# awslabs/dgl-ke

Hardware: NVIDIA H100
Metric: edges/sec TransE_l2 d=400 neg=200 at 1/2/4/8 H100 vs ref CPU; HBM GB/s %peak (higher is better)
Workload: dtype f32

## Files before the change

dgl-ke_b200/csrc/kge_fused.cu:

```cuda
#include <cuda.h>
#include <cstdio>
#include <cstdlib>
#include "kge_common.cuh"
#include "kge_tc.cuh"

namespace kge {

using namespace tc;

namespace {

constexpr int kTileM = 128;
constexpr int kThreadsF = 384;
constexpr int kProducerWarp = 8;
constexpr int kMaxS1 = 4, kMaxS2 = 8;
constexpr int kMaxPf = 8;
constexpr uint32_t kRingBytes = 192 * 1024;
constexpr int kWc = 128;
constexpr float kLog2e = 1.4426950408889634f;
constexpr float kLn2 = 0.6931471805599453f;

struct FusedArgs {
  int model, adversarial;
  float gamma, Tl2e, inv2B, uni;
  float reg_coef;
  int reg_norm;
  int C, Rx, Ry, D;
  int N1;
  int nblkD;
  int nS1, nS2;
  uint32_t stage1Bytes, stage2Bytes;
  float *VhiT, *VloT;
  float* colpart;
  int ncolpart;
  const float* x2;
  const float* y2;
  const float* pos;
  const float* wt;
  const float* wbar;
  float *gpos, *rowsum, *pl, *nl;
  float* dumpS;
  float* dumpV;
  const float *Xhi, *Xlo;
  const long long* xids;
  TableView xtab;
  const float* xraw;
  float* gsn;
  float* out;
  int pf_slots;
  int pf_parity;
  int pf_lag;
// ... 43 lines not shown
  };
  for (long long k = 0; k < n && k < S; ++k) load(k);
  const int L = g.pf_lag < S - 1 ? g.pf_lag : (S > 2 ? S - 2 : 1);
  for (long long k = 0; k < n; ++k) {
    const int s = (int)(k % S);
    mbar_wait(&pf_full[w][s], (uint32_t)((k / S) & 1));
    const long long v = vrow(k);
    float* dst = v < nU ? g.pf_nc + v * (long long)g.D : g.pf_bn + (v - nU) * (long long)g.D;
    const long long kr = k - L + S;
    const bool reload = k >= L && kr < n;
    if (reload && kr >= base + 32) { base += 32; ids_lo = ids_hi; ids_hi = fetch_ids(base + 32); }
    if (elect_one()) {
      bulk_s2g(dst, slots + (size_t)s * g.pf_row_bytes, g.pf_row_bytes);
      bulk_commit();
      if (reload) { if (L == 3) bulk_wait_read<3>(); else if (L == 2) bulk_wait_read<2>(); else bulk_wait_read<1>(); }
    }
    __syncwarp();
    if (reload) load(kr);
  }
  if (elect_one()) bulk_wait_all();
  __syncwarp();
}

template <int NV>
__global__ void __launch_bounds__(kThreadsF, 1)
k_fused_pos(const __grid_constant__ CUtensorMap mXh, const __grid_constant__ CUtensorMap mXl,
            const __grid_constant__ CUtensorMap mYh1, const __grid_constant__ CUtensorMap mYl1,
            const __grid_constant__ CUtensorMap mYh2, const __grid_constant__ CUtensorMap mYl2, FusedArgs g) {
  extern __shared__ __align__(1024) uint8_t smem_raw[];
  __shared__ __align__(8) uint64_t full1[kMaxS1], empty1[kMaxS1], full2[kMaxS2], empty2[kMaxS2];
  __shared__ __align__(8) uint64_t pf_full[2][kMaxPf];
  __shared__ __align__(16) float colA[NV];
  __shared__ __align__(16) float cpart[8][NV];

  const int warp = threadIdx.x >> 5, lane = threadIdx.x & 31;
  uint8_t* ring = (uint8_t*)(((uintptr_t)smem_raw + 1023) & ~(uintptr_t)1023);

  const int mtiles = (g.Rx + kTileM - 1) / kTileM;
  const int ntiles = g.C * mtiles;
  const int nkb1 = (g.D + 31) >> 5;
  const int nkb2 = (g.Ry + 31) >> 5;
  const int nchunks = (g.D + kWc - 1) / kWc;
  constexpr uint32_t yBytes1 = (uint32_t)NV * 128u;
  constexpr uint32_t yBytes2 = (uint32_t)kWc * 128u;
  const bool l2 = g.model == KGE_TRANSE_L2;

  if (threadIdx.x == 0) {
    for (int s = 0; s < kMaxS1; ++s) { mbar_init(&full1[s], 1); mbar_init(&empty1[s], 8); }
    for (int s = 0; s < kMaxS2; ++s) { mbar_init(&full2[s], 1); mbar_init(&empty2[s], 8); }
    for (int s = 0; s < kMaxPf; ++s) { mbar_init(&pf_full[0][s], 1); mbar_init(&pf_full[1][s], 1); }
    asm volatile("fence.mbarrier_init.release.cluster;" ::: "memory");
  }
  if (warp == kProducerWarp && lane == 0) {
    tma_prefetch_desc(&mXh); tma_prefetch_desc(&mXl); tma_prefetch_desc(&mYh1);
    tma_prefetch_desc(&mYl1); tma_prefetch_desc(&mYh2); tma_prefetch_desc(&mYl2);
  }
  __syncthreads();

  if (warp >= 8) {
  asm volatile("setmaxnreg.dec.sync.aligned.u32 56;");
  if (warp == kProducerWarp) {
    uint32_t n1 = 0, n2 = 0;
    for (int tile = blockIdx.x; tile < ntiles; tile += gridDim.x) {
      const int c = tile / mtiles, m0 = (tile % mtiles) * kTileM;
      for (uint32_t k = (n2 > (uint32_t)g.nS2 ? n2 - g.nS2 : 0); k < n2; ++k) mbar_wait(&empty2[k % g.nS2], (k / g.nS2) & 1);
      for (int kb = 0; kb < nkb1; ++kb, ++n1) {
        const uint32_t s = n1 % g.nS1;
        mbar_wait(&empty1[s], ((n1 / g.nS1) & 1) ^ 1);
        uint8_t* st = ring + (size_t)s * g.stage1Bytes;
        const int yx = (c * g.nblkD + kb) * g.Rx + m0;
        const int yy = (c * g.nblkD + kb) * g.Ry;
        if (elect_one()) {
          mbar_expect_tx(&full1[s], 2u * 16384u + 2u * yBytes1);
          tma_load_2d(st, &mXh, &full1[s], 0, yx);
          tma_load_2d(st + 16384, &mXl, &full1[s], 0, yx);
          tma_load_2d(st + 32768, &mYh1, &full1[s], 0, yy);
          tma_load_2d(st + 32768 + yBytes1, &mYl1, &full1[s], 0, yy);
        }
        __syncwarp();
      }
      for (uint32_t k = (n1 > (uint32_t)g.nS1 ? n1 - g.nS1 : 0); k < n1; ++k) mbar_wait(&empty1[k % g.nS1], (k / g.nS1) & 1);
      for (int ch = 0; ch < nchunks; ++ch) {
        for (int kb = 0; kb < nkb2; ++kb, ++n2) {
          const uint32_t s = n2 % g.nS2;
          mbar_wait(&empty2[s], ((n2 / g.nS2) & 1) ^ 1);
          uint8_t* st = ring + (size_t)s * g.stage2Bytes;
          const int yy = (c * nkb2 + kb) * g.D + ch * kWc;
          if (elect_one()) {
            mbar_expect_tx(&full2[s], 2u * yBytes2);
            tma_load_2d(st, &mYh2, &full2[s], 0, yy);
            tma_load_2d(st + yBytes2, &mYl2, &full2[s], 0, yy);
          }
          __syncwarp();
        }
      }
    }
  } else if (warp >= 10 && g.pf_slots > 0) {
    prefetch_rows(g, ring, pf_full, warp - 10, lane);
  }
  } else {
    asm volatile("setmaxnreg.inc.sync.aligned.u32 224;");
    const int wg = warp >> 2, q = lane & 3;
    const int et = threadIdx.x;
    const int rloc = wg * 64 + (warp & 3) * 16 + (lane >> 2);
    uint32_t n1 = 0, n2 = 0;
    float acc[NV / 2];
    for (int tile = blockIdx.x; tile < ntiles; tile += gridDim.x) {
      const int c = tile / mtiles, m0 = (tile % mtiles) * kTileM;
      epi_bar();
      for (int y = et; y < NV; y += 256) {
        const bool ok = y < g.Ry;
        colA[y] = (l2 && ok) ? g.y2[(long long)c * g.Ry + y] : 0.f;
      }
      epi_bar();
#pragma unroll
      for (int i = 0; i < NV / 2; ++i) acc[i] = 0.f;
      for (int kb = 0; kb < nkb1; ++kb, ++n1) {
        const uint32_t s = n1 % g.nS1;
        mbar_wait(&full1[s], (n1 / g.nS1) & 1);
        const uint32_t st = smem_u32(ring + (size_t)s * g.stage1Bytes);
        const uint64_t dXh = make_desc(st + wg * 8192u), dXl = make_desc(st + 16384u + wg * 8192u);
        const uint64_t dYh = make_desc(st + 32768u), dYl = make_desc(st + 32768u + yBytes1);
        const int kleft = g.D - kb * 32;
        const int ksteps = kleft >= 32 ? 4 : (kleft >> 3);
        wgmma_fence();
        for (int ks = 0; ks < ksteps; ++ks) {
          const uint64_t o = (uint64_t)(ks * 2);
          wgmma_ss<NV>(acc, dXh + o, dYh + o, 1u);
          wgmma_ss<NV>(acc, dXh + o, dYl + o, 1u);
          wgmma_ss<NV>(acc, dXl + o, dYh + o, 1u);
        }
        wgmma_commit();
        if (kb > 0) {
          wgmma_wait<1>();
          if (lane == 0) mbar_arrive(&empty1[(n1 - 1) % g.nS1]);
        }
      }
      wgmma_wait<0>();
      if (lane == 0) mbar_arrive(&empty1[(n1 - 1) % g.nS1]);
      reg_fence(acc);

      float rscal[2];
#pragma unroll
      for (int h = 0; h < 2; ++h) {
        const int m = m0 + rloc + 8 * h;
        const bool row_ok = m < g.Rx;
        const long long gx = (long long)c * g.Rx + (row_ok ? m : 0);
        const float x2v = (l2 && row_ok) ? g.x2[gx] : 0.f;
        const float w_i = (g.wt && row_ok) ? g.wt[gx] : 1.f;
        const float kw = w_i * g.inv2B;
        float mxl = -INFINITY;
        if (g.adversarial || g.dumpS) {
#pragma unroll
          for (int j = 0; j < NV / 8; ++j) {
            float sv[2];
#pragma unroll
            for (int e = 0; e < 2; ++e) {
              const int col = 8 * j + 2 * q + e;
              float s = acc[4 * j + 2 * h + e];
              if (l2) {
                const float sqc = fmaxf(fmaf(-2.f, s, colA[col]) + x2v, 1e-30f);
                s = g.gamma - sqc * rsqrta(sqc);
              }
              sv[e] = s;
              if (col < g.Ry) mxl = fmaxf(mxl, s * g.Tl2e);
// ... 12 lines not shown
#pragma unroll
        for (int j = 0; j < NV / 8; ++j) {
#pragma unroll
          for (int e = 0; e < 2; ++e) {
            const int col = 8 * j + 2 * q + e;
            float s = acc[4 * j + 2 * h + e], rinv = 1.f;
            if (l2) {
              const float sq = fmaf(-2.f, s, colA[col]) + x2v;
              const float sqc = fmaxf(sq, 1e-30f);
              const float r = rsqrta(sqc);
              s = g.gamma - sqc * r;
              rinv = (sq > 1e-30f) ? r : 0.f;
            }
            const float pe = g.adversarial ? ex2a(fmaf(s, g.Tl2e, -mxl)) : 1.f;
            const float t = ex2a(-fabsf(s) * kLog2e);
            const float u = 1.f + t;
            const float r1 = rcpa(u);
            const float sig = (s >= 0.f) ? r1 : t * r1;
            const float sp = fmaf(kLn2, lg2a(u), fmaxf(s, 0.f));
            const bool ok = row_ok && (col < g.Ry);
            const float coef = ok ? pe * sig * kw * rinv : 0.f;
            if (ok) { nls = fmaf(pe, sp, nls); den += pe; }
            rs += coef;
            acc[4 * j + 2 * h + e] = coef;
          }
        }
        den += __shfl_xor_sync(0xffffffffu, den, 1); den += __shfl_xor_sync(0xffffffffu, den, 2);
        nls += __shfl_xor_sync(0xffffffffu, nls, 1); nls += __shfl_xor_sync(0xffffffffu, nls, 2);
        rs += __shfl_xor_sync(0xffffffffu, rs, 1); rs += __shfl_xor_sync(0xffffffffu, rs, 2);
        const float rscale = g.adversarial ? (row_ok ? 1.f / den : 0.f) : g.uni;
        rscal[h] = rscale;
        if (g.dumpV && row_ok) {
#pragma unroll
          for (int j = 0; j < NV / 8; ++j)
            if (8 * j + 2 * q < g.Ry)
              *reinterpret_cast<float2*>(g.dumpV + gx * g.Ry + 8 * j + 2 * q) =
                  make_float2(acc[4 * j + 2 * h] * rscale, acc[4 * j + 2 * h + 1] * rscale);
        }
        {
          float* vh = g.VhiT + slabT_off(c, g.Rx, g.Ry, m, 0);
          float* vl = g.VloT + slabT_off(c, g.Rx, g.Ry, m, 0);
#pragma unroll
          for (int j = 0; j < NV / 8; ++j) {
#pragma unroll
            for (int e = 0; e < 2; ++e) {
              const int col = 8 * j + 2 * q + e;
              const float v = acc[4 * j + 2 * h + e] * rscale;
              if (row_ok && col < g.Ry) {
                float hi, lo;
                split_tf32(v, hi, lo);
                vh[col * 32] = hi; vl[col * 32] = lo;
              }
              if (l2) {
                float s = v;
                s += __shfl_xor_sync(0xffffffffu, s, 4);
                s += __shfl_xor_sync(0xffffffffu, s, 8);
                s += __shfl_xor_sync(0xffffffffu, s, 16);
                if (lane < 4) cpart[warp][col] = h ? cpart[warp][col] + s : s;
              }
            }
          }
        }
        if (q == 0 && row_ok) {
          const float ps = g.pos[gx];
          const float wb = g.wt ? *g.wbar : 1.f;
          g.pl[gx] = softplusf(-ps);
          g.nl[gx] = nls * rscale * w_i;
          g.gpos[gx] = -sigmoidf(-ps) * wb * g.inv2B;
          if (l2) g.rowsum[gx] = rs * rscale;
        }
      }
      if (l2) {
        epi_bar();
        float* dst = g.colpart + (long long)(tile % mtiles) * g.C * g.Ry + (long long)c * g.Ry;
        for (int y = et; y < g.Ry; y += 256) {
          float s = cpart[0][y];
#pragma unroll
          for (int w = 1; w < 8; ++w) s += cpart[w][y];
          dst[y] = s;
        }
      }
      {
        const int srcLo = (lane & ~3) | (q >> 1), srcHi = srcLo + 2;
        const bool odd = q & 1;
#pragma unroll
        for (int j = 0; j < NV / 8; ++j) {
          float o[4];
#pragma unroll
          for (int h = 0; h < 2; ++h) {
            const float v0 = acc[4 * j + 2 * h], v1 = acc[4 * j + 2 * h + 1];
            const float a0 = __shfl_sync(0xffffffffu, v0, srcLo), a1 = __shfl_sync(0xffffffffu, v1, srcLo);
            const float b0 = __shfl_sync(0xffffffffu, v0, srcHi), b1 = __shfl_sync(0xffffffffu, v1, srcHi);
            o[h] = odd ? a1 : a0;
            o[2 + h] = odd ? b1 : b0;
          }
          acc[4 * j + 0] = o[0]; acc[4 * j + 1] = o[1]; acc[4 * j + 2] = o[2]; acc[4 * j + 3] = o[3];
        }
      }

      for (int ch = 0; ch < nchunks; ++ch) {
        const int d0 = ch * kWc;
        float acc2[kWc / 2];
#pragma unroll
        for (int i = 0; i < kWc / 2; ++i) acc2[i] = 0.f;
#pragma unroll
        for (int kb = 0; kb < (NV + 31) / 32; ++kb) {
          if (kb >= nkb2) break;
          const uint32_t s = n2 % g.nS2;
          mbar_wait(&full2[s], (n2 / g.nS2) & 1);
          const uint32_t st = smem_u32(ring + (size_t)s * g.stage2Bytes);
          const uint64_t dYh = make_desc(st), dYl = make_desc(st + yBytes2);
          const int kleft = g.Ry - kb * 32;
          const int ksteps = kleft >= 32 ? 4 : (kleft >> 3);
          uint32_t ah[2][4] = {}, al[2][4] = {};
#pragma unroll
          for (int ks = 0; ks < 4; ++ks) {
            const int j = kb * 4 + ks;
            if (j < NV / 8 && ks < ksteps) {
              if (ks >= 2) wgmma_wait<1>();
#pragma unroll
              for (int r = 0; r < 4; ++r) {
                float hi, lo;
                split_tf32(acc[4 * j + r], hi, lo);
                ah[ks & 1][r] = __float_as_uint(hi); al[ks & 1][r] = __float_as_uint(lo);
              }
              wgmma_fence();
              const uint64_t o = (uint64_t)(ks * 2);
              wgmma_rs<kWc>(acc2, ah[ks & 1], dYh + o, 1u);
              wgmma_rs<kWc>(acc2, ah[ks & 1], dYl + o, 1u);
              wgmma_rs<kWc>(acc2, al[ks & 1], dYh + o, 1u);
              wgmma_commit();
              if (ks >= 1) { reg_fence(ah[(ks - 1) & 1]); reg_fence(al[(ks - 1) & 1]); }
            }
          }
          wgmma_wait<0>();
          reg_fence(ah[0]); reg_fence(ah[1]); reg_fence(al[0]); reg_fence(al[1]);
          if (lane == 0) mbar_arrive(&empty2[s]);
          ++n2;
        }
        reg_fence(acc2);
#pragma unroll
        for (int h = 0; h < 2; ++h) {
          const int m = m0 + rloc + 8 * h;
          if (m >= g.Rx) continue;
          float* orow = g.out + ((long long)c * g.Rx + m) * (long long)g.D;
#pragma unroll
          for (int j = 0; j < kWc / 8; ++j) {
            const int k = d0 + 8 * j + 2 * q;
            if (k >= g.D) continue;
            *reinterpret_cast<float2*>(orow + k) = make_float2(acc2[4 * j + 2 * h] * rscal[h], acc2[4 * j + 2 * h + 1] * rscal[h]);
          }
        }
      }
    }
  }
}

template <int NW, int KS>
__device__ __forceinline__ void neg_kblock(float (&acc)[NW / 2], uint64_t dVh, uint64_t dVl, uint64_t dAh, uint64_t dAl) {
  wgmma_fence();
#pragma unroll
  for (int ks = 0; ks < KS; ++ks) {
    const uint64_t o = (uint64_t)(ks * 2);
    wgmma_ss<NW>(acc, dVh + o, dAh + o, 1u);
    wgmma_ss<NW>(acc, dVh + o, dAl + o, 1u);
    wgmma_ss<NW>(acc, dVl + o, dAh + o, 1u);
  }
  wgmma_commit();
}

constexpr int kNegEpiLoads = 16;

template <int NW, bool FLAT>
__global__ void __launch_bounds__(kThreadsF, 1)
k_fused_neg(const __grid_constant__ CUtensorMap mVh, const __grid_constant__ CUtensorMap mVl,
            const __grid_constant__ CUtensorMap mAh, const __grid_constant__ CUtensorMap mAl, FusedArgs g) {
  extern __shared__ __align__(1024) uint8_t smem_raw[];
  __shared__ __align__(8) uint64_t full[kMaxS1], empty[kMaxS1];
  __shared__ __align__(8) uint64_t pf_full[2][kMaxPf];

  const int warp = threadIdx.x >> 5, lane = threadIdx.x & 31;
  uint8_t* ring = (uint8_t*)(((uintptr_t)smem_raw + 1023) & ~(uintptr_t)1023);

  const int mtiles = (g.Rx + kTileM - 1) / kTileM;
  const int ntiles = g.C * mtiles;
  const int nkb = (g.Ry + 31) >> 5;
  const int nch = (g.D + NW - 1) / NW;
  constexpr uint32_t aBytes = (uint32_t)kTileM * 128u;
  constexpr uint32_t bBytes = (uint32_t)NW * 128u;
  const bool l2 = g.model == KGE_TRANSE_L2;

// ... 86 lines not shown
            bh[jj] = __ldg(reinterpret_cast<const float2*>(brow[h] + k));
          } else {
            const long long so = boff[h] + (k >> 5) * blk + (k & 31);
            bh[jj] = __ldg(reinterpret_cast<const float2*>(g.Xhi + so));
            bl[jj] = __ldg(reinterpret_cast<const float2*>(g.Xlo + so));
          }
        }
      };
      float gsq[2] = {0.f, 0.f};
      for (int ch = 0; ch < nch; ++ch) {
        const int d0 = ch * NW;
        float acc[NW / 2];
#pragma unroll
        for (int i = 0; i < NW / 2; ++i) acc[i] = 0.f;
        for (int kb = 0; kb < nkb; ++kb, ++n) {
          const uint32_t s = n % g.nS1;
          mbar_wait(&full[s], (n / g.nS1) & 1);
          const uint32_t st = smem_u32(ring + (size_t)s * g.stage1Bytes);
          const uint64_t dVh = make_desc(st + wg * 8192u), dVl = make_desc(st + aBytes + wg * 8192u);
          const uint64_t dAh = make_desc(st + 2 * aBytes), dAl = make_desc(st + 2 * aBytes + bBytes);
          const int kleft = g.Ry - kb * 32;
          const int ksteps = kleft >= 32 ? 4 : (kleft >> 3);
          switch (ksteps) {
            case 4: neg_kblock<NW, 4>(acc, dVh, dVl, dAh, dAl); break;
            case 3: neg_kblock<NW, 3>(acc, dVh, dVl, dAh, dAl); break;
            case 2: neg_kblock<NW, 2>(acc, dVh, dVl, dAh, dAl); break;
            default: neg_kblock<NW, 1>(acc, dVh, dVl, dAh, dAl); break;
          }
          if (kb > 0) {
            wgmma_wait<1>();
            if (lane == 0) mbar_arrive(&empty[(n - 1) % g.nS1]);
          }
        }
        if (early) load_b(0, d0, 0);
        wgmma_wait<0>();
        if (lane == 0) mbar_arrive(&empty[(n - 1) % g.nS1]);
        reg_fence(acc);
#pragma unroll
        for (int h = 0; h < 2; ++h) {
          if (!rok[h]) continue;
          float* orow = g.out + ((long long)c * g.Rx + m0 + rloc + 8 * h) * (long long)g.D;
#pragma unroll
          for (int j0 = 0; j0 < NJ; j0 += NB) {
            if (!early || h > 0 || j0 > 0) load_b(h, d0, j0);
#pragma unroll
            for (int jj = 0; jj < NB; ++jj) {
              const int j = j0 + jj;
              const int k = d0 + 8 * j + 2 * q;
              if (j >= NJ || k >= g.D) continue;
              float o0 = acc[4 * j + 2 * h], o1 = acc[4 * j + 2 * h + 1];
// ... 6 lines not shown
            }
          }
        }
      }
#pragma unroll
      for (int h = 0; h < 2; ++h) {
        float v = gsq[h];
        v += __shfl_xor_sync(0xffffffffu, v, 1);
        v += __shfl_xor_sync(0xffffffffu, v, 2);
        const int m = m0 + rloc + 8 * h;
        if (q == 0 && m < g.Rx) g.gsn[(long long)c * g.Rx + m] = v / (float)g.D;
      }
    }
  }
}

}

bool fused_supported(const StepParams& p) {
  return umma_supported(p) && !p.hinge && !p.pairwise && !p.neg_deg && p.Cs <= 240 && p.Ns <= 240;
}

namespace {
struct Geometry { int Rx, Ry, N1, nS1, nS2, pf_slots; uint32_t stage1Bytes, stage2Bytes, pf_off; bool ok; };

int neg_chunk_width(int D, bool want_prefetch) {
  static const int widths[] = {64, 128, 200, 256};
  int best = 0;
  long long best_rows = 0;
  for (int w : widths) {
    if (w == 256 && want_prefetch) continue;
    const long long rows = (long long)((D + w - 1) / w) * (kTileM + w);
    if (!best || rows < best_rows) { best = w; best_rows = rows; }
  }
  return best;
}

Geometry geometry(const StepParams& p, int mode, bool want_prefetch) {
  Geometry q{};
  const uint32_t row = (uint32_t)p.D * 4u;
  if (mode == 1) {
    q.Rx = p.Ns; q.Ry = p.Cs;
    q.N1 = neg_chunk_width(p.D, want_prefetch);
    q.stage1Bytes = 2u * kTileM * 128u + 2u * (uint32_t)q.N1 * 128u;
    q.nS1 = (int)(kRingBytes / q.stage1Bytes); if (q.nS1 > kMaxS1) q.nS1 = kMaxS1;
    q.ok = q.nS1 >= 2;
    if (q.ok && want_prefetch) {
      int nS = q.nS1;
      while (nS > 2 && kRingBytes - (uint32_t)nS * q.stage1Bytes < 2u * kMaxPf * row) --nS;
      const uint32_t used = (uint32_t)nS * q.stage1Bytes;
      int slots = (int)((kRingBytes - used) / (2u * row));
      if (slots > kMaxPf) slots = kMaxPf;
      if (slots >= 2) { q.pf_slots = slots; q.nS1 = nS; q.pf_off = used; }
    }
    return q;
  }
  q.Rx = p.Cs; q.Ry = p.Ns;
  q.N1 = q.Ry <= 64 ? 64 : (q.Ry <= 128 ? 128 : (q.Ry <= 208 ? 208 : 256));
  q.stage1Bytes = 2u * 16384u + 2u * (uint32_t)q.N1 * 128u;
  q.stage2Bytes = 2u * (uint32_t)kWc * 128u;
  q.nS1 = (int)(kRingBytes / q.stage1Bytes); if (q.nS1 > kMaxS1) q.nS1 = kMaxS1;
  q.nS2 = (int)(kRingBytes / q.stage2Bytes); if (q.nS2 > kMaxS2) q.nS2 = kMaxS2;
  q.ok = q.nS1 >= 2 && q.nS2 >= 2;
  if (q.ok && want_prefetch) {
    int nS1 = q.nS1, nS2 = q.nS2;
    uint32_t want = 2u * kMaxPf * row;
    while (nS1 > 2 && kRingBytes - (uint32_t)nS1 * q.stage1Bytes < want) --nS1;
    uint32_t used = (uint32_t)nS1 * q.stage1Bytes;
    if (want > kRingBytes - used) want = kRingBytes - used;
    while (nS2 > 4 && kRingBytes - (uint32_t)nS2 * q.stage2Bytes < want) --nS2;
    if ((uint32_t)nS2 * q.stage2Bytes > used) used = (uint32_t)nS2 * q.stage2Bytes;
    int slots = (int)((kRingBytes - used) / (2u * row));
    if (slots > kMaxPf) slots = kMaxPf;
    if (slots >= 2) { q.pf_slots = slots; q.nS1 = nS1; q.nS2 = nS2; q.pf_off = used; }
  }
  return q;
}

int launch_error() {
  const cudaError_t e = cudaGetLastError();
  return e == cudaSuccess ? KGE_OK : fail(KGE_ERR_CUDA, "k_fused launch: %s", cudaGetErrorString(e));
}
template <int NV>
int launch_pos(const LaunchCtx& c, int grid, size_t smem, const CUtensorMap* m, const FusedArgs& g) {
  if (int rc = smem_optin((const void*)k_fused_pos<NV>, smem)) return rc;
  KGE_LAUNCH_NAMED(c, "k_fused<P: S=A.Bn^T, loss, GA=V.Bn>", (k_fused_pos<NV>), grid, kThreadsF, smem,
                   m[0], m[1], m[2], m[3], m[4], m[5], g);
  return launch_error();
}
template <int NW, bool FLAT>
int launch_neg_src(const LaunchCtx& c, int grid, size_t smem, const CUtensorMap* m, const FusedArgs& g) {
  if (int rc = smem_optin((const void*)k_fused_neg<NW, FLAT>, smem)) return rc;
  KGE_LAUNCH_NAMED(c, "k_fused<N: G_neg=V^T.A, mean sq>", (k_fused_neg<NW, FLAT>), grid, kThreadsF, smem, m[0], m[1], m[2], m[3], g);
  return launch_error();
}
template <int NW>
int launch_neg(const LaunchCtx& c, int grid, size_t smem, const CUtensorMap* m, const FusedArgs& g) {
  return (g.xraw || g.xids) ? launch_neg_src<NW, true>(c, grid, smem, m, g) : launch_neg_src<NW, false>(c, grid, smem, m, g);
}
int launch_width(const LaunchCtx& c, bool P, int grid, size_t smem, const CUtensorMap* m, const FusedArgs& g) {
  switch (g.N1) {
    case 64: return P ? launch_pos<64>(c, grid, smem, m, g) : launch_neg<64>(c, grid, smem, m, g);
    case 128: return P ? launch_pos<128>(c, grid, smem, m, g) : launch_neg<128>(c, grid, smem, m, g);
    case 200: return launch_neg<200>(c, grid, smem, m, g);
    case 208: return launch_pos<208>(c, grid, smem, m, g);
    default: return P ? launch_pos<256>(c, grid, smem, m, g) : launch_neg<256>(c, grid, smem, m, g);
  }
}
}

int fused_prefetch_slots(const StepParams& p, int mode) { return geometry(p, mode, true).pf_slots; }

int fused_launch(const LaunchCtx& c, const StepParams& p, const StepWs& w, int mode, const float* wt, float* dumpS,
                 float* dumpV, const TableView* ent, const long long* neg_ids, const FusedPrefetch* pf) {
  FusedArgs g{};
  g.model = p.model; g.adversarial = p.adversarial;
  g.gamma = p.gamma; g.Tl2e = p.adv_temperature * kLog2e; g.inv2B = 0.5f / (float)p.B; g.uni = 1.f / (float)p.Ns;
  g.reg_coef = p.reg_coef; g.reg_norm = p.reg_norm;
  g.C = p.C; g.D = p.D; g.nblkD = slab_blocks(p.D);
  const bool P = mode == 0;
  const Geometry q = geometry(p, mode, pf != nullptr && ent != nullptr);
  if (!q.ok) return fail(KGE_ERR_UNSUPPORTED, "fused kernel: shape does not fit (N1=%d)", q.N1);
  g.Rx = q.Rx; g.Ry = q.Ry; g.N1 = q.N1; g.nS1 = q.nS1; g.nS2 = q.nS2;
  g.stage1Bytes = q.stage1Bytes; g.stage2Bytes = q.stage2Bytes;
  if (pf && ent && q.pf_slots >= 2) {
    static const int lag_env = getenv("KGE_B200_PF_LAG") ? atoi(getenv("KGE_B200_PF_LAG")) : 1;
    g.pf_lag = lag_env < 1 ? 1 : (lag_env > 3 ? 3 : lag_env);
    g.pf_slots = q.pf_slots; g.pf_off = q.pf_off; g.pf_row_bytes = (uint32_t)p.D * 4u; g.pf_parity = mode;
    g.pf_node_ids = pf->node_ids; g.pf_nU_dev = pf->nU_dev; g.pf_nU = pf->nU; g.pf_nNeg = pf->nNeg;
    g.pf_neg_ids = pf->neg_ids; g.pf_nc = pf->nc; g.pf_bn = pf->bn;
    g.xtab = *ent;
  }
  g.VhiT = w.VhiT; g.VloT = w.VloT; g.colpart = w.colpart; g.ncolpart = (p.Cs + kTileM - 1) / kTileM;
  g.dumpV = dumpV;
  const size_t smem = kRingBytes + 1024;
  const int mtiles = (g.Rx + kTileM - 1) / kTileM;
  int grid = p.C * mtiles;
  if (grid > c.num_sms) grid = c.num_sms;
  CUtensorMap m[6];
  if (P) {
    g.x2 = w.a2; g.y2 = w.b2;
    g.pos = w.pos; g.wt = wt; g.wbar = w.wbar;
    g.gpos = w.gpos; g.rowsum = w.rowsum; g.pl = w.pl; g.nl = w.nl;
    g.dumpS = dumpS;
    g.out = w.GA;
    const long long rowsX = (long long)p.C * p.Cs * g.nblkD, rowsY = (long long)p.C * p.Ns * g.nblkD;
    const long long rowsYT = (long long)p.C * slab_blocks(p.Ns) * p.D;
    if (tc_make_map(&m[0], w.Ahi, rowsX, 32, kTileM) || tc_make_map(&m[1], w.Alo, rowsX, 32, kTileM) ||
        tc_make_map(&m[2], w.Bhi, rowsY, 32, g.N1) || tc_make_map(&m[3], w.Blo, rowsY, 32, g.N1) ||
        tc_make_map(&m[4], w.BhiT, rowsYT, 32, kWc) || tc_make_map(&m[5], w.BloT, rowsYT, 32, kWc))
      return KGE_ERR_CUDA;
    return launch_width(c, true, grid, smem, m, g);
  }
  g.Xhi = w.Bhi; g.Xlo = w.Blo;
  if (ent && ent->n_shards == 1 && neg_ids) { g.xids = neg_ids; g.xtab = *ent; }
  if (w.BnRaw) g.xraw = w.BnRaw;
  g.gsn = w.gsn;
  g.out = w.Bn;
  const long long rowsV = (long long)p.C * slab_blocks(p.Cs) * p.Ns, rowsA = (long long)p.C * slab_blocks(p.Cs) * p.D;
  if (tc_make_map(&m[0], w.VhiT, rowsV, 32, kTileM) || tc_make_map(&m[1], w.VloT, rowsV, 32, kTileM) ||
      tc_make_map(&m[2], w.AhiT, rowsA, 32, g.N1) || tc_make_map(&m[3], w.AloT, rowsA, 32, g.N1))
    return KGE_ERR_CUDA;
  return launch_width(c, false, grid, smem, m, g);
}

}
```

dgl-ke_b200/csrc/kge_tc.cuh:

```cuda
#pragma once
#include <cuda.h>
#include <cuda_runtime.h>
#include <stdint.h>

namespace kge {
namespace tc {

__device__ __forceinline__ uint32_t smem_u32(const void* p) { return (uint32_t)__cvta_generic_to_shared(p); }

__device__ __forceinline__ bool elect_one() {
  uint32_t pred = 0;
  asm volatile(
      "{\n\t.reg .pred P1;\n\t"
      "elect.sync _|P1, 0xFFFFFFFF;\n\t"
      "selp.b32 %0, 1, 0, P1;\n\t}"
      : "=r"(pred));
  return pred != 0;
}

__device__ __forceinline__ void mbar_init(uint64_t* bar, uint32_t count) {
  asm volatile("mbarrier.init.shared::cta.b64 [%0], %1;" ::"r"(smem_u32(bar)), "r"(count));
}
__device__ __forceinline__ void mbar_expect_tx(uint64_t* bar, uint32_t bytes) {
  asm volatile("mbarrier.arrive.expect_tx.shared::cta.b64 _, [%0], %1;" ::"r"(smem_u32(bar)), "r"(bytes) : "memory");
// ... 72 lines not shown
               : "l"(adesc), "l"(bdesc), "r"(accumulate));
}
template <>
__device__ __forceinline__ void wgmma_ss<208>(float (&d)[104], uint64_t adesc, uint64_t bdesc, uint32_t accumulate) {
  asm volatile("{\n\t.reg .pred p;\n\tsetp.ne.b32 p, %106, 0;\n\t"
               "wgmma.mma_async.sync.aligned.m64n208k8.f32.tf32.tf32 {%0,%1,%2,%3,%4,%5,%6,%7,%8,%9,%10,%11,%12,%13,%14,%15,%16,%17,%18,%19,%20,%21,%22,%23,%24,%25,%26,%27,%28,%29,%30,%31,%32,%33,%34,%35,%36,%37,%38,%39,%40,%41,%42,%43,%44,%45,%46,%47,%48,%49,%50,%51,%52,%53,%54,%55,%56,%57,%58,%59,%60,%61,%62,%63,%64,%65,%66,%67,%68,%69,%70,%71,%72,%73,%74,%75,%76,%77,%78,%79,%80,%81,%82,%83,%84,%85,%86,%87,%88,%89,%90,%91,%92,%93,%94,%95,%96,%97,%98,%99,%100,%101,%102,%103}, %104, %105, p, 1, 1;\n\t}"
               : KGE_D32(0), KGE_D32(32), KGE_D32(64), KGE_D4(96), KGE_D4(100)
               : "l"(adesc), "l"(bdesc), "r"(accumulate));
}
template <>
__device__ __forceinline__ void wgmma_ss<256>(float (&d)[128], uint64_t adesc, uint64_t bdesc, uint32_t accumulate) {
  asm volatile("{\n\t.reg .pred p;\n\tsetp.ne.b32 p, %130, 0;\n\t"
               "wgmma.mma_async.sync.aligned.m64n256k8.f32.tf32.tf32 {%0,%1,%2,%3,%4,%5,%6,%7,%8,%9,%10,%11,%12,%13,%14,%15,%16,%17,%18,%19,%20,%21,%22,%23,%24,%25,%26,%27,%28,%29,%30,%31,%32,%33,%34,%35,%36,%37,%38,%39,%40,%41,%42,%43,%44,%45,%46,%47,%48,%49,%50,%51,%52,%53,%54,%55,%56,%57,%58,%59,%60,%61,%62,%63,%64,%65,%66,%67,%68,%69,%70,%71,%72,%73,%74,%75,%76,%77,%78,%79,%80,%81,%82,%83,%84,%85,%86,%87,%88,%89,%90,%91,%92,%93,%94,%95,%96,%97,%98,%99,%100,%101,%102,%103,%104,%105,%106,%107,%108,%109,%110,%111,%112,%113,%114,%115,%116,%117,%118,%119,%120,%121,%122,%123,%124,%125,%126,%127}, %128, %129, p, 1, 1;\n\t}"
               : KGE_D32(0), KGE_D32(32), KGE_D32(64), KGE_D32(96)
               : "l"(adesc), "l"(bdesc), "r"(accumulate));
}
template <>
__device__ __forceinline__ void wgmma_rs<128>(float (&d)[64], const uint32_t (&a)[4], uint64_t bdesc, uint32_t accumulate) {
  asm volatile("{\n\t.reg .pred p;\n\tsetp.ne.b32 p, %69, 0;\n\t"
               "wgmma.mma_async.sync.aligned.m64n128k8.f32.tf32.tf32 {%0,%1,%2,%3,%4,%5,%6,%7,%8,%9,%10,%11,%12,%13,%14,%15,%16,%17,%18,%19,%20,%21,%22,%23,%24,%25,%26,%27,%28,%29,%30,%31,%32,%33,%34,%35,%36,%37,%38,%39,%40,%41,%42,%43,%44,%45,%46,%47,%48,%49,%50,%51,%52,%53,%54,%55,%56,%57,%58,%59,%60,%61,%62,%63}, {%64,%65,%66,%67}, %68, p, 1, 1;\n\t}"
               : KGE_D32(0), KGE_D32(32)
               : "r"(a[0]), "r"(a[1]), "r"(a[2]), "r"(a[3]), "l"(bdesc), "r"(accumulate));
}
#undef KGE_D4
#undef KGE_D16
#undef KGE_D32

__device__ __forceinline__ uint64_t make_desc(uint32_t saddr) {
  uint64_t d = 0;
  d |= (uint64_t)((saddr >> 4) & 0x3FFF);
  d |= (uint64_t)1 << 16;
  d |= (uint64_t)(1024 >> 4) << 32;
  d |= (uint64_t)1 << 62;
  return d;
}

__device__ __forceinline__ float ex2a(float x) { float y; asm("ex2.approx.ftz.f32 %0, %1;" : "=f"(y) : "f"(x)); return y; }
__device__ __forceinline__ float lg2a(float x) { float y; asm("lg2.approx.ftz.f32 %0, %1;" : "=f"(y) : "f"(x)); return y; }
__device__ __forceinline__ float rcpa(float x) { float y; asm("rcp.approx.ftz.f32 %0, %1;" : "=f"(y) : "f"(x)); return y; }
__device__ __forceinline__ float rsqrta(float x) { float y; asm("rsqrt.approx.ftz.f32 %0, %1;" : "=f"(y) : "f"(x)); return y; }
__device__ __forceinline__ float sqrta(float x) { float y; asm("sqrt.approx.ftz.f32 %0, %1;" : "=f"(y) : "f"(x)); return y; }

}

int tc_make_map(CUtensorMap* m, const float* base, long long rows, long long cols, int box_rows);

// ... 2 lines not shown
```

Measured before the change: 29.44 million.

## Stage V tile in shared memory, offload V export to handoff warps, add n200 second GEMM

The positive-side fused kernel now writes the softmax coefficient matrix V into a swizzled shared-memory buffer instead of holding it in registers. Dedicated handoff warps then export the hi/lo split of V to global memory and reduce the column sums, overlapping that work with the second GEMM. The second GEMM reads its A fragments from shared memory and can use an N=200 chunk width when that wastes less padding for D (e.g. D=400). The ring buffer grows when prefetch is off, and a vfree barrier gates reuse of the V buffer. The change adds shared-memory traffic and a new cross-warp synchronisation, and it leaves fewer pipeline stages for the V buffer.

```diff
diff --git a/dgl-ke_b200/csrc/kge_fused.cu b/dgl-ke_b200/csrc/kge_fused.cu
--- a/dgl-ke_b200/csrc/kge_fused.cu
+++ b/dgl-ke_b200/csrc/kge_fused.cu
@@ -1,6 +1,7 @@
 #include <cuda.h>
 #include <cstdio>
 #include <cstdlib>
+#include <mutex>
 #include "kge_common.cuh"
 #include "kge_tc.cuh"
 
@@ -13,10 +14,11 @@
 constexpr int kTileM = 128;
 constexpr int kThreadsF = 384;
 constexpr int kProducerWarp = 8;
+constexpr int kHandoffWarp = 9;
 constexpr int kMaxS1 = 4, kMaxS2 = 8;
 constexpr int kMaxPf = 8;
 constexpr uint32_t kRingBytes = 192 * 1024;
-constexpr int kWc = 128;
+constexpr uint32_t kRingBytesP = 223 * 1024;
 constexpr float kLog2e = 1.4426950408889634f;
 constexpr float kLn2 = 0.6931471805599453f;
 
@@ -27,6 +29,7 @@
   int reg_norm;
   int C, Rx, Ry, D;
   int N1;
+  int N2;
   int nblkD;
   int nS1, nS2;
   uint32_t stage1Bytes, stage2Bytes;
@@ -116,32 +119,83 @@
   __syncwarp();
 }
 
+template <int NW, int KS>
+__device__ __forceinline__ void kblock_3xtf32(float (&acc)[NW / 2], uint64_t dXh, uint64_t dXl, uint64_t dYh, uint64_t dYl) {
+  wgmma_fence();
+#pragma unroll
+  for (int ks = 0; ks < KS; ++ks) {
+    const uint64_t o = (uint64_t)(ks * 2);
+    wgmma_ss<NW>(acc, dXh + o, dYh + o, 1u);
+    wgmma_ss<NW>(acc, dXh + o, dYl + o, 1u);
+    wgmma_ss<NW>(acc, dXl + o, dYh + o, 1u);
+  }
+  wgmma_commit();
+}
+
 template <int NV>
+__device__ __forceinline__ int vsm_idx(int i, int k) {
+  const int g = i & 7, h = (i >> 3) & 1, kk = k & 7;
+  const int L = 4 * g + (kk & 3);
+  return (((i >> 4) * (NV / 8) + (k >> 3)) * 32 + (L ^ ((L >> 3) & 3))) * 4 + h + 2 * (kk >> 2);
+}
+
+template <int NW>
+__device__ __forceinline__ void pos_kstep(float (&acc2)[NW / 2], uint32_t (&ah)[4], uint32_t (&al)[4], const float* vf,
+                                          uint64_t dYh, uint64_t dYl) {
+  const float4 v = *reinterpret_cast<const float4*>(vf);
+  const float a[4] = {v.x, v.y, v.z, v.w};
+#pragma unroll
+  for (int r = 0; r < 4; ++r) {
+    float hi, lo;
+    split_tf32(a[r], hi, lo);
+    ah[r] = __float_as_uint(hi); al[r] = __float_as_uint(lo);
+  }
+  wgmma_fence();
+  wgmma_rs<NW>(acc2, ah, dYh, 1u);
+  wgmma_rs<NW>(acc2, ah, dYl, 1u);
+  wgmma_rs<NW>(acc2, al, dYh, 1u);
+  wgmma_commit();
+}
+
+__device__ __forceinline__ int tile_row() {
+  uint32_t t;
+  asm volatile("mov.u32 %0, %%tid.x;" : "=r"(t));
+  return (int)((t >> 5) * 16 + ((t >> 2) & 7));
+}
+
+template <int NV, int NW>
 __global__ void __launch_bounds__(kThreadsF, 1)
 k_fused_pos(const __grid_constant__ CUtensorMap mXh, const __grid_constant__ CUtensorMap mXl,
             const __grid_constant__ CUtensorMap mYh1, const __grid_constant__ CUtensorMap mYl1,
             const __grid_constant__ CUtensorMap mYh2, const __grid_constant__ CUtensorMap mYl2, FusedArgs g) {
   extern __shared__ __align__(1024) uint8_t smem_raw[];
   __shared__ __align__(8) uint64_t full1[kMaxS1], empty1[kMaxS1], full2[kMaxS2], empty2[kMaxS2];
+  __shared__ __align__(8) uint64_t vfree;
   __shared__ __align__(8) uint64_t pf_full[2][kMaxPf];
   __shared__ __align__(16) float colA[NV];
-  __shared__ __align__(16) float cpart[8][NV];
+  __shared__ float rsc[kTileM];
 
   const int warp = threadIdx.x >> 5, lane = threadIdx.x & 31;
   uint8_t* ring = (uint8_t*)(((uintptr_t)smem_raw + 1023) & ~(uintptr_t)1023);
+  float* vsm = reinterpret_cast<float*>(ring);
+  constexpr uint32_t vBytes = (uint32_t)NV * 512u;
+  uint8_t* ring2 = ring + vBytes;
 
   const int mtiles = (g.Rx + kTileM - 1) / kTileM;
   const int ntiles = g.C * mtiles;
   const int nkb1 = (g.D + 31) >> 5;
   const int nkb2 = (g.Ry + 31) >> 5;
-  const int nchunks = (g.D + kWc - 1) / kWc;
+  const int nchunks = (g.D + NW - 1) / NW;
   constexpr uint32_t yBytes1 = (uint32_t)NV * 128u;
-  constexpr uint32_t yBytes2 = (uint32_t)kWc * 128u;
+  constexpr uint32_t yBytes2 = (uint32_t)NW * 128u;
   const bool l2 = g.model == KGE_TRANSE_L2;
+  const int nhand = g.pf_slots > 0 ? 1 : 3;
+  const uint32_t hand_bar_n = 256u + 32u * (uint32_t)nhand;
 
   if (threadIdx.x == 0) {
     for (int s = 0; s < kMaxS1; ++s) { mbar_init(&full1[s], 1); mbar_init(&empty1[s], 8); }
     for (int s = 0; s < kMaxS2; ++s) { mbar_init(&full2[s], 1); mbar_init(&empty2[s], 8); }
+    mbar_init(&vfree, 8 + nhand);
     for (int s = 0; s < kMaxPf; ++s) { mbar_init(&pf_full[0][s], 1); mbar_init(&pf_full[1][s], 1); }
     asm volatile("fence.mbarrier_init.release.cluster;" ::: "memory");
   }
@@ -154,10 +208,10 @@
   if (warp >= 8) {
   asm volatile("setmaxnreg.dec.sync.aligned.u32 56;");
   if (warp == kProducerWarp) {
-    uint32_t n1 = 0, n2 = 0;
-    for (int tile = blockIdx.x; tile < ntiles; tile += gridDim.x) {
+    uint32_t n1 = 0, n2 = 0, it = 0;
+    for (int tile = blockIdx.x; tile < ntiles; tile += gridDim.x, ++it) {
       const int c = tile / mtiles, m0 = (tile % mtiles) * kTileM;
-      for (uint32_t k = (n2 > (uint32_t)g.nS2 ? n2 - g.nS2 : 0); k < n2; ++k) mbar_wait(&empty2[k % g.nS2], (k / g.nS2) & 1);
+      if (it > 0) mbar_wait(&vfree, (it - 1) & 1);
       for (int kb = 0; kb < nkb1; ++kb, ++n1) {
         const uint32_t s = n1 % g.nS1;
         mbar_wait(&empty1[s], ((n1 / g.nS1) & 1) ^ 1);
@@ -178,8 +232,8 @@
         for (int kb = 0; kb < nkb2; ++kb, ++n2) {
           const uint32_t s = n2 % g.nS2;
           mbar_wait(&empty2[s], ((n2 / g.nS2) & 1) ^ 1);
-          uint8_t* st = ring + (size_t)s * g.stage2Bytes;
-          const int yy = (c * nkb2 + kb) * g.D + ch * kWc;
+          uint8_t* st = ring2 + (size_t)s * g.stage2Bytes;
+          const int yy = (c * nkb2 + kb) * g.D + ch * NW;
           if (elect_one()) {
             mbar_expect_tx(&full2[s], 2u * yBytes2);
             tma_load_2d(st, &mYh2, &full2[s], 0, yy);
@@ -189,6 +243,43 @@
         }
       }
     }
+  } else if (warp - kHandoffWarp < nhand) {
+    const int hw = warp - kHandoffWarp;
+    for (int tile = blockIdx.x; tile < ntiles; tile += gridDim.x) {
+      const int c = tile / mtiles, m0 = (tile % mtiles) * kTileM;
+      const int rows = g.Rx - m0 < kTileM ? g.Rx - m0 : kTileM;
+      const int nb = (rows + 31) >> 5;
+      asm volatile("bar.sync 2, %0;" ::"r"(hand_bar_n) : "memory");
+      float* dst = g.colpart + (long long)(tile % mtiles) * g.C * g.Ry + (long long)c * g.Ry;
+      for (int j = hw; j < g.Ry; j += nhand) {
+        float s = 0.f;
+        float v[kTileM / 32];
+#pragma unroll
+        for (int b = 0; b < kTileM / 32; ++b) {
+          const int i = 32 * b + lane;
+          v[b] = b < nb ? vsm[vsm_idx<NV>(i, j)] * rsc[i] : 0.f;
+        }
+#pragma unroll
+        for (int b = 0; b < kTileM / 32; ++b) {
+          const int i = 32 * b + lane;
+          if (i < rows) {
+            float hi, lo;
+            split_tf32(v[b], hi, lo);
+            const long long o = slabT_off(c, g.Rx, g.Ry, m0 + i, j);
+            g.VhiT[o] = hi; g.VloT[o] = lo;
+          }
+          s += v[b];
+        }
+        if (l2) {
+#pragma unroll
+          for (int x = 16; x >= 1; x >>= 1) s += __shfl_xor_sync(0xffffffffu, s, x);
+          if (lane == 0) dst[j] = s;
+        }
+      }
+      asm volatile("fence.proxy.async.shared::cta;" ::: "memory");
+      __syncwarp();
+      if (lane == 0) mbar_arrive(&vfree);
+    }
   } else if (warp >= 10 && g.pf_slots > 0) {
     prefetch_rows(g, ring, pf_full, warp - 10, lane);
   }
@@ -196,9 +287,7 @@
     asm volatile("setmaxnreg.inc.sync.aligned.u32 224;");
     const int wg = warp >> 2, q = lane & 3;
     const int et = threadIdx.x;
-    const int rloc = wg * 64 + (warp & 3) * 16 + (lane >> 2);
     uint32_t n1 = 0, n2 = 0;
-    float acc[NV / 2];
     for (int tile = blockIdx.x; tile < ntiles; tile += gridDim.x) {
       const int c = tile / mtiles, m0 = (tile % mtiles) * kTileM;
       epi_bar();
@@ -207,6 +296,9 @@
         colA[y] = (l2 && ok) ? g.y2[(long long)c * g.Ry + y] : 0.f;
       }
       epi_bar();
+      float rscal[2];
+      {
+      float acc[NV / 2];
 #pragma unroll
       for (int i = 0; i < NV / 2; ++i) acc[i] = 0.f;
       for (int kb = 0; kb < nkb1; ++kb, ++n1) {
@@ -217,14 +309,12 @@
         const uint64_t dYh = make_desc(st + 32768u), dYl = make_desc(st + 32768u + yBytes1);
         const int kleft = g.D - kb * 32;
         const int ksteps = kleft >= 32 ? 4 : (kleft >> 3);
-        wgmma_fence();
-        for (int ks = 0; ks < ksteps; ++ks) {
-          const uint64_t o = (uint64_t)(ks * 2);
-          wgmma_ss<NV>(acc, dXh + o, dYh + o, 1u);
-          wgmma_ss<NV>(acc, dXh + o, dYl + o, 1u);
-          wgmma_ss<NV>(acc, dXl + o, dYh + o, 1u);
-        }
-        wgmma_commit();
+        switch (ksteps) {
+          case 4: kblock_3xtf32<NV, 4>(acc, dXh, dXl, dYh, dYl); break;
+          case 3: kblock_3xtf32<NV, 3>(acc, dXh, dXl, dYh, dYl); break;
+          case 2: kblock_3xtf32<NV, 2>(acc, dXh, dXl, dYh, dYl); break;
+          default: kblock_3xtf32<NV, 1>(acc, dXh, dXl, dYh, dYl); break;
+        }
         if (kb > 0) {
           wgmma_wait<1>();
           if (lane == 0) mbar_arrive(&empty1[(n1 - 1) % g.nS1]);
@@ -233,8 +323,9 @@
       wgmma_wait<0>();
       if (lane == 0) mbar_arrive(&empty1[(n1 - 1) % g.nS1]);
       reg_fence(acc);
-
-      float rscal[2];
+      epi_bar();
+      const int rloc = tile_row();
+
 #pragma unroll
       for (int h = 0; h < 2; ++h) {
         const int m = m0 + rloc + 8 * h;
@@ -293,7 +384,7 @@
             const float coef = ok ? pe * sig * kw * rinv : 0.f;
             if (ok) { nls = fmaf(pe, sp, nls); den += pe; }
             rs += coef;
-            acc[4 * j + 2 * h + e] = coef;
+            vsm[vsm_idx<NV>(rloc + 8 * h, col)] = coef;
           }
         }
         den += __shfl_xor_sync(0xffffffffu, den, 1); den += __shfl_xor_sync(0xffffffffu, den, 2);
@@ -302,35 +393,11 @@
         const float rscale = g.adversarial ? (row_ok ? 1.f / den : 0.f) : g.uni;
         rscal[h] = rscale;
         if (g.dumpV && row_ok) {
-#pragma unroll
           for (int j = 0; j < NV / 8; ++j)
             if (8 * j + 2 * q < g.Ry)
               *reinterpret_cast<float2*>(g.dumpV + gx * g.Ry + 8 * j + 2 * q) =
-                  make_float2(acc[4 * j + 2 * h] * rscale, acc[4 * j + 2 * h + 1] * rscale);
-        }
-        {
-          float* vh = g.VhiT + slabT_off(c, g.Rx, g.Ry, m, 0);
-          float* vl = g.VloT + slabT_off(c, g.Rx, g.Ry, m, 0);
-#pragma unroll
-          for (int j = 0; j < NV / 8; ++j) {
-#pragma unroll
-            for (int e = 0; e < 2; ++e) {
-              const int col = 8 * j + 2 * q + e;
-              const float v = acc[4 * j + 2 * h + e] * rscale;
-              if (row_ok && col < g.Ry) {
-                float hi, lo;
-                split_tf32(v, hi, lo);
-                vh[col * 32] = hi; vl[col * 32] = lo;
-              }
-              if (l2) {
-                float s = v;
-                s += __shfl_xor_sync(0xffffffffu, s, 4);
-                s += __shfl_xor_sync(0xffffffffu, s, 8);
-                s += __shfl_xor_sync(0xffffffffu, s, 16);
-                if (lane < 4) cpart[warp][col] = h ? cpart[warp][col] + s : s;
-              }
-            }
-          }
+                  make_float2(vsm[vsm_idx<NV>(rloc + 8 * h, 8 * j + 2 * q)] * rscale,
+                              vsm[vsm_idx<NV>(rloc + 8 * h, 8 * j + 2 * q + 1)] * rscale);
         }
         if (q == 0 && row_ok) {
           const float ps = g.pos[gx];
@@ -341,74 +408,45 @@
           if (l2) g.rowsum[gx] = rs * rscale;
         }
       }
-      if (l2) {
-        epi_bar();
-        float* dst = g.colpart + (long long)(tile % mtiles) * g.C * g.Ry + (long long)c * g.Ry;
-        for (int y = et; y < g.Ry; y += 256) {
-          float s = cpart[0][y];
-#pragma unroll
-          for (int w = 1; w < 8; ++w) s += cpart[w][y];
-          dst[y] = s;
-        }
-      }
-      {
-        const int srcLo = (lane & ~3) | (q >> 1), srcHi = srcLo + 2;
-        const bool odd = q & 1;
-#pragma unroll
-        for (int j = 0; j < NV / 8; ++j) {
-          float o[4];
-#pragma unroll
-          for (int h = 0; h < 2; ++h) {
-            const float v0 = acc[4 * j + 2 * h], v1 = acc[4 * j + 2 * h + 1];
-            const float a0 = __shfl_sync(0xffffffffu, v0, srcLo), a1 = __shfl_sync(0xffffffffu, v1, srcLo);
-            const float b0 = __shfl_sync(0xffffffffu, v0, srcHi), b1 = __shfl_sync(0xffffffffu, v1, srcHi);
-            o[h] = odd ? a1 : a0;
-            o[2 + h] = odd ? b1 : b0;
-          }
-          acc[4 * j + 0] = o[0]; acc[4 * j + 1] = o[1]; acc[4 * j + 2] = o[2]; acc[4 * j + 3] = o[3];
-        }
-      }
-
+      if (q == 0) { rsc[rloc] = rscal[0]; rsc[rloc + 8] = rscal[1]; }
+      }
+      asm volatile("bar.arrive 2, %0;" ::"r"(hand_bar_n) : "memory");
+      __syncwarp();
+
+      const float* vw = vsm + ((warp * (NV / 8)) * 32 + (lane ^ ((lane >> 3) & 3))) * 4;
+      const int rloc = tile_row();
       for (int ch = 0; ch < nchunks; ++ch) {
-        const int d0 = ch * kWc;
-        float acc2[kWc / 2];
-#pragma unroll
-        for (int i = 0; i < kWc / 2; ++i) acc2[i] = 0.f;
-#pragma unroll
-        for (int kb = 0; kb < (NV + 31) / 32; ++kb) {
-          if (kb >= nkb2) break;
+        const int d0 = ch * NW;
+        float acc2[NW / 2];
+#pragma unroll
+        for (int i = 0; i < NW / 2; ++i) acc2[i] = 0.f;
+        uint32_t ah[2][4], al[2][4];
+#pragma unroll 1
+        for (int kb = 0; kb < nkb2; ++kb) {
           const uint32_t s = n2 % g.nS2;
           mbar_wait(&full2[s], (n2 / g.nS2) & 1);
-          const uint32_t st = smem_u32(ring + (size_t)s * g.stage2Bytes);
+          const uint32_t st = smem_u32(ring2 + (size_t)s * g.stage2Bytes);
           const uint64_t dYh = make_desc(st), dYl = make_desc(st + yBytes2);
           const int kleft = g.Ry - kb * 32;
           const int ksteps = kleft >= 32 ? 4 : (kleft >> 3);
-          uint32_t ah[2][4] = {}, al[2][4] = {};
 #pragma unroll
           for (int ks = 0; ks < 4; ++ks) {
             const int j = kb * 4 + ks;
-            if (j < NV / 8 && ks < ksteps) {
-              if (ks >= 2) wgmma_wait<1>();
-#pragma unroll
-              for (int r = 0; r < 4; ++r) {
-                float hi, lo;
-                split_tf32(acc[4 * j + r], hi, lo);
-                ah[ks & 1][r] = __float_as_uint(hi); al[ks & 1][r] = __float_as_uint(lo);
+            if (ks < ksteps) {
+              const uint64_t o = (uint64_t)(ks * 2);
+              pos_kstep<NW>(acc2, ah[j & 1], al[j & 1], vw + j * 128, dYh + o, dYl + o);
+              if (j > 0) {
+                wgmma_wait<1>();
+                reg_fence(ah[(j - 1) & 1]); reg_fence(al[(j - 1) & 1]);
+                if (ks == 0 && lane == 0) mbar_arrive(&empty2[(n2 - 1) % g.nS2]);
               }
-              wgmma_fence();
-              const uint64_t o = (uint64_t)(ks * 2);
-              wgmma_rs<kWc>(acc2, ah[ks & 1], dYh + o, 1u);
-              wgmma_rs<kWc>(acc2, ah[ks & 1], dYl + o, 1u);
-              wgmma_rs<kWc>(acc2, al[ks & 1], dYh + o, 1u);
-              wgmma_commit();
-              if (ks >= 1) { reg_fence(ah[(ks - 1) & 1]); reg_fence(al[(ks - 1) & 1]); }
             }
           }
-          wgmma_wait<0>();
-          reg_fence(ah[0]); reg_fence(ah[1]); reg_fence(al[0]); reg_fence(al[1]);
-          if (lane == 0) mbar_arrive(&empty2[s]);
           ++n2;
         }
+        wgmma_wait<0>();
+        reg_fence(ah[0]); reg_fence(ah[1]); reg_fence(al[0]); reg_fence(al[1]);
+        if (lane == 0) mbar_arrive(&empty2[(n2 - 1) % g.nS2]);
         reg_fence(acc2);
 #pragma unroll
         for (int h = 0; h < 2; ++h) {
@@ -416,28 +454,18 @@
           if (m >= g.Rx) continue;
           float* orow = g.out + ((long long)c * g.Rx + m) * (long long)g.D;
 #pragma unroll
-          for (int j = 0; j < kWc / 8; ++j) {
+          for (int j = 0; j < NW / 8; ++j) {
             const int k = d0 + 8 * j + 2 * q;
             if (k >= g.D) continue;
             *reinterpret_cast<float2*>(orow + k) = make_float2(acc2[4 * j + 2 * h] * rscal[h], acc2[4 * j + 2 * h + 1] * rscal[h]);
           }
         }
       }
+      asm volatile("fence.proxy.async.shared::cta;" ::: "memory");
+      __syncwarp();
+      if (lane == 0) mbar_arrive(&vfree);
     }
   }
-}
-
-template <int NW, int KS>
-__device__ __forceinline__ void neg_kblock(float (&acc)[NW / 2], uint64_t dVh, uint64_t dVl, uint64_t dAh, uint64_t dAl) {
-  wgmma_fence();
-#pragma unroll
-  for (int ks = 0; ks < KS; ++ks) {
-    const uint64_t o = (uint64_t)(ks * 2);
-    wgmma_ss<NW>(acc, dVh + o, dAh + o, 1u);
-    wgmma_ss<NW>(acc, dVh + o, dAl + o, 1u);
-    wgmma_ss<NW>(acc, dVl + o, dAh + o, 1u);
-  }
-  wgmma_commit();
 }
 
 constexpr int kNegEpiLoads = 16;
@@ -570,10 +598,10 @@
           const int kleft = g.Ry - kb * 32;
           const int ksteps = kleft >= 32 ? 4 : (kleft >> 3);
           switch (ksteps) {
-            case 4: neg_kblock<NW, 4>(acc, dVh, dVl, dAh, dAl); break;
-            case 3: neg_kblock<NW, 3>(acc, dVh, dVl, dAh, dAl); break;
-            case 2: neg_kblock<NW, 2>(acc, dVh, dVl, dAh, dAl); break;
-            default: neg_kblock<NW, 1>(acc, dVh, dVl, dAh, dAl); break;
+            case 4: kblock_3xtf32<NW, 4>(acc, dVh, dVl, dAh, dAl); break;
+            case 3: kblock_3xtf32<NW, 3>(acc, dVh, dVl, dAh, dAl); break;
+            case 2: kblock_3xtf32<NW, 2>(acc, dVh, dVl, dAh, dAl); break;
+            default: kblock_3xtf32<NW, 1>(acc, dVh, dVl, dAh, dAl); break;
           }
           if (kb > 0) {
             wgmma_wait<1>();
@@ -626,7 +654,7 @@
 }
 
 namespace {
-struct Geometry { int Rx, Ry, N1, nS1, nS2, pf_slots; uint32_t stage1Bytes, stage2Bytes, pf_off; bool ok; };
+struct Geometry { int Rx, Ry, N1, N2, nS1, nS2, pf_slots; uint32_t ringBytes, stage1Bytes, stage2Bytes, pf_off; bool ok; };
 
 int neg_chunk_width(int D, bool want_prefetch) {
   static const int widths[] = {64, 128, 200, 256};
@@ -645,6 +673,7 @@
   const uint32_t row = (uint32_t)p.D * 4u;
   if (mode == 1) {
     q.Rx = p.Ns; q.Ry = p.Cs;
+    q.ringBytes = kRingBytes;
     q.N1 = neg_chunk_width(p.D, want_prefetch);
     q.stage1Bytes = 2u * kTileM * 128u + 2u * (uint32_t)q.N1 * 128u;
     q.nS1 = (int)(kRingBytes / q.stage1Bytes); if (q.nS1 > kMaxS1) q.nS1 = kMaxS1;
@@ -661,36 +690,69 @@
   }
   q.Rx = p.Cs; q.Ry = p.Ns;
   q.N1 = q.Ry <= 64 ? 64 : (q.Ry <= 128 ? 128 : (q.Ry <= 208 ? 208 : 256));
+  const uint32_t ring = want_prefetch ? kRingBytes : kRingBytesP;
+  q.ringBytes = ring;
   q.stage1Bytes = 2u * 16384u + 2u * (uint32_t)q.N1 * 128u;
-  q.stage2Bytes = 2u * (uint32_t)kWc * 128u;
-  q.nS1 = (int)(kRingBytes / q.stage1Bytes); if (q.nS1 > kMaxS1) q.nS1 = kMaxS1;
-  q.nS2 = (int)(kRingBytes / q.stage2Bytes); if (q.nS2 > kMaxS2) q.nS2 = kMaxS2;
-  q.ok = q.nS1 >= 2 && q.nS2 >= 2;
-  if (q.ok && want_prefetch) {
-    int nS1 = q.nS1, nS2 = q.nS2;
-    uint32_t want = 2u * kMaxPf * row;
-    while (nS1 > 2 && kRingBytes - (uint32_t)nS1 * q.stage1Bytes < want) --nS1;
-    uint32_t used = (uint32_t)nS1 * q.stage1Bytes;
-    if (want > kRingBytes - used) want = kRingBytes - used;
-    while (nS2 > 4 && kRingBytes - (uint32_t)nS2 * q.stage2Bytes < want) --nS2;
-    if ((uint32_t)nS2 * q.stage2Bytes > used) used = (uint32_t)nS2 * q.stage2Bytes;
-    int slots = (int)((kRingBytes - used) / (2u * row));
+  int nS1 = (int)(ring / q.stage1Bytes); if (nS1 > kMaxS1) nS1 = kMaxS1;
+  if (nS1 < 2) return q;
+  const uint32_t vBytes = (uint32_t)q.N1 * 512u;
+  const bool w200 = (p.D + 199) / 200 * 200 < (p.D + 127) / 128 * 128;
+  const int widths[2] = {w200 ? 200 : 128, w200 ? 128 : 200};
+  Geometry first{};
+  for (int NW : widths) {
+    Geometry t = q;
+    t.N2 = NW;
+    t.stage2Bytes = 2u * (uint32_t)NW * 128u;
+    if (vBytes + 2u * t.stage2Bytes > ring) continue;
+    t.nS1 = nS1;
+    t.nS2 = (int)((ring - vBytes) / t.stage2Bytes); if (t.nS2 > kMaxS2) t.nS2 = kMaxS2;
+    t.ok = true;
+    if (!want_prefetch) return t;
+    if (!first.ok) first = t;
+    const uint32_t want = 2u * kMaxPf * row;
+    int s1 = t.nS1, s2 = t.nS2;
+    while (s1 > 2 && ring - (uint32_t)s1 * q.stage1Bytes < want) --s1;
+    while (s2 > 2 && ring - (vBytes + (uint32_t)s2 * t.stage2Bytes) < want) --s2;
+    uint32_t used = (uint32_t)s1 * q.stage1Bytes;
+    if (vBytes + (uint32_t)s2 * t.stage2Bytes > used) used = vBytes + (uint32_t)s2 * t.stage2Bytes;
+    int slots = (int)((ring - used) / (2u * row));
     if (slots > kMaxPf) slots = kMaxPf;
-    if (slots >= 2) { q.pf_slots = slots; q.nS1 = nS1; q.nS2 = nS2; q.pf_off = used; }
-  }
-  return q;
+    if (slots >= 2) { t.pf_slots = slots; t.nS1 = s1; t.nS2 = s2; t.pf_off = used; return t; }
+  }
+  return first;
 }
 
 int launch_error() {
   const cudaError_t e = cudaGetLastError();
   return e == cudaSuccess ? KGE_OK : fail(KGE_ERR_CUDA, "k_fused launch: %s", cudaGetErrorString(e));
 }
+const char* pos_launch_name(int NV, int NW, int pf) {
+  static const int nvs[4] = {64, 128, 208, 256}, nws[2] = {128, 200};
+  static char names[4][2][kMaxPf + 1][96];
+  static std::once_flag once;
+  std::call_once(once, [] {
+    for (int a = 0; a < 4; ++a)
+      for (int b = 0; b < 2; ++b)
+        for (int f = 0; f <= kMaxPf; ++f)
+          snprintf(names[a][b][f], sizeof(names[a][b][f]), "k_fused<P: S=A.Bn^T, loss, GA=V.Bn> NV=%d NW=%d pf=%d hand=%d",
+                   nvs[a], nws[b], f, f > 0 ? 1 : 3);
+  });
+  const int a = NV == 64 ? 0 : NV == 128 ? 1 : NV == 208 ? 2 : 3;
+  return names[a][NW == 200][pf < 0 ? 0 : (pf > kMaxPf ? kMaxPf : pf)];
+}
+template <int NV, int NW>
+int launch_pos(const LaunchCtx& c, int grid, size_t smem, const CUtensorMap* m, const FusedArgs& g) {
+  if (int rc = smem_optin((const void*)k_fused_pos<NV, NW>, smem)) return rc;
+  KGE_LAUNCH_NAMED(c, pos_launch_name(NV, NW, g.pf_slots), (k_fused_pos<NV, NW>), grid, kThreadsF, smem,
+                   m[0], m[1], m[2], m[3], m[4], m[5], g);
+  return launch_error();
+}
 template <int NV>
 int launch_pos(const LaunchCtx& c, int grid, size_t smem, const CUtensorMap* m, const FusedArgs& g) {
-  if (int rc = smem_optin((const void*)k_fused_pos<NV>, smem)) return rc;
-  KGE_LAUNCH_NAMED(c, "k_fused<P: S=A.Bn^T, loss, GA=V.Bn>", (k_fused_pos<NV>), grid, kThreadsF, smem,
-                   m[0], m[1], m[2], m[3], m[4], m[5], g);
-  return launch_error();
+  if constexpr (NV < 256) {
+    if (g.N2 == 200) return launch_pos<NV, 200>(c, grid, smem, m, g);
+  }
+  return launch_pos<NV, 128>(c, grid, smem, m, g);
 }
 template <int NW, bool FLAT>
 int launch_neg_src(const LaunchCtx& c, int grid, size_t smem, const CUtensorMap* m, const FusedArgs& g) {
@@ -725,7 +787,7 @@
   const bool P = mode == 0;
   const Geometry q = geometry(p, mode, pf != nullptr && ent != nullptr);
   if (!q.ok) return fail(KGE_ERR_UNSUPPORTED, "fused kernel: shape does not fit (N1=%d)", q.N1);
-  g.Rx = q.Rx; g.Ry = q.Ry; g.N1 = q.N1; g.nS1 = q.nS1; g.nS2 = q.nS2;
+  g.Rx = q.Rx; g.Ry = q.Ry; g.N1 = q.N1; g.N2 = q.N2; g.nS1 = q.nS1; g.nS2 = q.nS2;
   g.stage1Bytes = q.stage1Bytes; g.stage2Bytes = q.stage2Bytes;
   if (pf && ent && q.pf_slots >= 2) {
     static const int lag_env = getenv("KGE_B200_PF_LAG") ? atoi(getenv("KGE_B200_PF_LAG")) : 1;
@@ -737,7 +799,7 @@
   }
   g.VhiT = w.VhiT; g.VloT = w.VloT; g.colpart = w.colpart; g.ncolpart = (p.Cs + kTileM - 1) / kTileM;
   g.dumpV = dumpV;
-  const size_t smem = kRingBytes + 1024;
+  const size_t smem = q.ringBytes + 1024;
   const int mtiles = (g.Rx + kTileM - 1) / kTileM;
   int grid = p.C * mtiles;
   if (grid > c.num_sms) grid = c.num_sms;
@@ -752,7 +814,7 @@
     const long long rowsYT = (long long)p.C * slab_blocks(p.Ns) * p.D;
     if (tc_make_map(&m[0], w.Ahi, rowsX, 32, kTileM) || tc_make_map(&m[1], w.Alo, rowsX, 32, kTileM) ||
         tc_make_map(&m[2], w.Bhi, rowsY, 32, g.N1) || tc_make_map(&m[3], w.Blo, rowsY, 32, g.N1) ||
-        tc_make_map(&m[4], w.BhiT, rowsYT, 32, kWc) || tc_make_map(&m[5], w.BloT, rowsYT, 32, kWc))
+        tc_make_map(&m[4], w.BhiT, rowsYT, 32, g.N2) || tc_make_map(&m[5], w.BloT, rowsYT, 32, g.N2))
       return KGE_ERR_CUDA;
     return launch_width(c, true, grid, smem, m, g);
   }
diff --git a/dgl-ke_b200/csrc/kge_tc.cuh b/dgl-ke_b200/csrc/kge_tc.cuh
--- a/dgl-ke_b200/csrc/kge_tc.cuh
+++ b/dgl-ke_b200/csrc/kge_tc.cuh
@@ -118,6 +118,13 @@
                : KGE_D32(0), KGE_D32(32)
                : "r"(a[0]), "r"(a[1]), "r"(a[2]), "r"(a[3]), "l"(bdesc), "r"(accumulate));
 }
+template <>
+__device__ __forceinline__ void wgmma_rs<200>(float (&d)[100], const uint32_t (&a)[4], uint64_t bdesc, uint32_t accumulate) {
+  asm volatile("{\n\t.reg .pred p;\n\tsetp.ne.b32 p, %105, 0;\n\t"
+               "wgmma.mma_async.sync.aligned.m64n200k8.f32.tf32.tf32 {%0,%1,%2,%3,%4,%5,%6,%7,%8,%9,%10,%11,%12,%13,%14,%15,%16,%17,%18,%19,%20,%21,%22,%23,%24,%25,%26,%27,%28,%29,%30,%31,%32,%33,%34,%35,%36,%37,%38,%39,%40,%41,%42,%43,%44,%45,%46,%47,%48,%49,%50,%51,%52,%53,%54,%55,%56,%57,%58,%59,%60,%61,%62,%63,%64,%65,%66,%67,%68,%69,%70,%71,%72,%73,%74,%75,%76,%77,%78,%79,%80,%81,%82,%83,%84,%85,%86,%87,%88,%89,%90,%91,%92,%93,%94,%95,%96,%97,%98,%99}, {%100,%101,%102,%103}, %104, p, 1, 1;\n\t}"
+               : KGE_D32(0), KGE_D32(32), KGE_D32(64), KGE_D4(96)
+               : "r"(a[0]), "r"(a[1]), "r"(a[2]), "r"(a[3]), "l"(bdesc), "r"(accumulate));
+}
 #undef KGE_D4
 #undef KGE_D16
 #undef KGE_D32
```

Result: faster. 31.21 million (median of 6 runs) (+6.0%).
